# HKU-BAL/Clair3-RNA

Measured on AMD Instinct MI355X. Metric: candidate sites/sec (tensor build + inference), higher is better.
Workload: dtype f16 hi/lo split x3, f32 accumulate (fp32-equivalent); 1 GPU; synthetic ONT dRNA004 chr20 ~20x (BASELINE.json configs[1]); contig_len=64444167, chunks=13, channels=18, precision=f16x3, reads_per_rank=53937, exonic_bp_per_rank=1936903, parallelism=chunks sharded by contig, 1 rank(s), no collective, streams=2

## Files before the change

### clair3_rna_amd/csrc/net_kernels.hpp

```cpp
#pragma once
#include <hip/hip_runtime.h>
#include <mutex>
#include <chrono>
#include <type_traits>
#include <stdint.h>

#include <cmath>
#include <cstring>
#include <functional>
#include <string>
#include <vector>

#include "../../include/c3r.h"

namespace c3r {

typedef float floatx16 __attribute__((ext_vector_type(16)));
typedef float floatx4 __attribute__((ext_vector_type(4)));

constexpr int NET_H1 = 128;
constexpr int NET_H2 = 160;
constexpr int NET_T = C3R_WINDOW;
constexpr int NET_SITES = 32;
constexpr int LSTM_SB = 2;
constexpr int LSTM_SITES = NET_SITES * LSTM_SB;
#ifndef C3R_W8_PD
#define C3R_W8_PD 1
#endif
#ifndef C3R_W8_MAP
#define C3R_W8_MAP 0
#endif
#ifndef C3R_W8_PRIO
#define C3R_W8_PRIO 0
#endif
#ifndef C3R_DIR_ILV
#define C3R_DIR_ILV 1
#endif
constexpr int NET_FLAT = NET_T * 2 * NET_H2;
constexpr int NET_L4 = 128;

__device__ __forceinline__ float fast_sigmoid(float x) {
    return __builtin_amdgcn_rcpf(1.0f + __builtin_amdgcn_exp2f(-1.4426950408889634f * x));
}
__device__ __forceinline__ float fast_tanh(float x) {
    return fmaf(2.0f, __builtin_amdgcn_rcpf(1.0f + __builtin_amdgcn_exp2f(-2.8853900817779268f * x)), -1.0f);
}
__device__ __forceinline__ float gate_frac(float a, float b) {
    const float t = 1.0f + a;
    const float r = __builtin_amdgcn_rcpf(fmaf(t, b, t));
    return fmaf(-b, r, r);
}
__device__ __forceinline__ float selu(float x) {
    const float scale = 1.0507009873554805f, alpha = 1.6732632423543772f;
    return x > 0.f ? scale * x : scale * alpha * (__expf(x) - 1.0f);
}

template <int INP, int CIN, int H, bool INT_IN, int SB = 2, int ABL = 0>
__global__ __launch_bounds__(256, (SB == 1 ? 2 : 1)) void k_lstm(const void *__restrict__ xin, const float4 *__restrict__ Wp,
                                                                  const float *__restrict__ bp, float *__restrict__ y, int n,
                                                                  const int32_t *__restrict__ row_idx = nullptr ,
                                                                  int x16 = 0 ) {
    constexpr int NGX = INP / 8;
    constexpr int NGH = H / 8;
    constexpr int NG = NGX + NGH;
    constexpr int HP = H + 4;
    constexpr int NBLK = 4 * H / 32;
    constexpr int NT = NBLK / 4;
    constexpr int WG_SITES = 32 * SB;
    static_assert(INP % 16 == 0 && H % 32 == 0, "shape: even k-group counts for the ping-pong pipeline");
    __shared__ __attribute__((aligned(16))) float hbuf[2][WG_SITES][HP];

    const int tid = threadIdx.x, lane = tid & 63, wave = tid >> 6;
    const int j = lane & 31, hh = lane >> 5;
    const int dir = blockIdx.y;
    const int site0 = blockIdx.x * WG_SITES;

    const float4 *wl = Wp + ((size_t)(dir * 4 + wave) * NG) * NT * 64 + lane;
    float bias_a[NT];
#pragma unroll
    for (int tt = 0; tt < NT; ++tt) bias_a[tt] = hh == 0 ? bp[((size_t)dir * NBLK + wave * NT + tt) * 32 + j] : 0.f;

    float cst[NT][SB][4];
#pragma unroll
    for (int tt = 0; tt < NT; ++tt)
// ... 167 lines not shown
#define C3R_W8_ASYNC 1
#endif
__device__ __forceinline__ void lds_arrive(int *c) {
    __builtin_amdgcn_fence(__ATOMIC_RELEASE, "workgroup");
    if ((threadIdx.x & 63) == 0) atomicAdd(c, 1);
}
__device__ __forceinline__ void lds_wait(int *c, int target, int *tmo) {
    for (int it = 0; __atomic_load_n(c, __ATOMIC_RELAXED) < target; ++it) {
        if (it >= (1 << 24)) { if ((threadIdx.x & 63) == 0 && tmo) atomicOr(tmo, 1); break; }
        __builtin_amdgcn_s_sleep(1);
    }
    __builtin_amdgcn_fence(__ATOMIC_ACQUIRE, "workgroup");
}

#ifndef C3R_PROBE_Y1
#define C3R_PROBE_Y1 0
#endif
__host__ __device__ constexpr int w16_bias_row(int st, int q, int m) { return 8 * ((2 * q + st) & 3) + 4 * ((2 * q + st) >> 2) + m; }
template <int ABL = 0, bool RTS = false>
__global__ __launch_bounds__(512, 2) void k_lstm2_w16(const _Float16 *__restrict__ xin, const half8 *__restrict__ Wp,
                                                       const float *__restrict__ bp, int n, const half8 *__restrict__ W4p,
                                                       float *__restrict__ a4part, int nstride, float wsc_arg = WSCALE, float wun_arg = WUNSCALE, float wun4_arg = WUNSCALE,
                                                       int *tmo = nullptr ) {
    const float wsc = RTS ? wsc_arg : WSCALE, wun = RTS ? wun_arg : WUNSCALE, wun4 = RTS ? wun4_arg : WUNSCALE;
    constexpr int INP = 2 * NET_H1, H = NET_H2, NGX = INP / 32, NGH = H / 32, NG = NGX + NGH, NU = 2 * NG, HP = H + 8, NBLK = 4 * H / 32, NTQ = NBLK / 4;
    constexpr int SB = 4, WG_SITES = 16 * SB, KC = INP / 8, PD = C3R_W8_PD;
    static_assert(NTQ == 5 && NU == 26 && PD == 1, "3 + 2 tile split of a quarter, 26 (k-group, subtile) units, one unit of prefetch");
    __shared__ __attribute__((aligned(16))) _Float16 hb_hi[2][WG_SITES][HP];
    __shared__ __attribute__((aligned(16))) _Float16 hb_lo[2][WG_SITES][HP];
    __shared__ __attribute__((aligned(16))) _Float16 xs[2][KC][WG_SITES][8];
    __shared__ __attribute__((aligned(16))) float s_bias[NBLK][2][16];
    __shared__ int s_ctr[4];

    const int tid = threadIdx.x, lane = tid & 63, wave = tid >> 6;
    const int c16 = lane & 15, q4 = lane >> 4;
    const int sq = C3R_W8_MAP ? (wave >> 1) : (wave & 3);
    const bool heavy3 = C3R_W8_MAP ? !(wave & 1) : (wave < 4);
    const int dir = C3R_DIR_ILV ? blockIdx.x : blockIdx.y;
    const int site0 = (C3R_DIR_ILV ? blockIdx.y : blockIdx.x) * WG_SITES;
    const int ns = nstride ? nstride : n;
    const size_t plane_in = (size_t)ns * NET_T * INP;

    for (int i = tid; i < WG_SITES * HP; i += 512) { (&hb_hi[0][0][0])[i] = (_Float16)0.f; (&hb_lo[0][0][0])[i] = (_Float16)0.f; }
    for (int i = tid; i < NBLK * 32; i += 512) {
        const int T = i >> 5, st = (i >> 4) & 1, q = (i >> 2) & 3, m = i & 3;
        s_bias[T][st][4 * q + m] = wsc * bp[((size_t)dir * NBLK + T) * 32 + w16_bias_row(st, q, m)];
    }
    if (tid < 4) s_ctr[tid] = 0;

    int xsite = site0 + lane;
    if (xsite >= n) xsite = n - 1;
    auto dma_x = [&](int tt_) {
        typedef const _Float16 __attribute__((address_space(1))) *gp_t;
        typedef _Float16 __attribute__((address_space(3))) *lp_t;
#pragma unroll
        for (int r = 0; r < 2 * KC / 8; ++r) {
            const int row = wave * (2 * KC / 8) + r, pl = row / KC, kc = row % KC;
            const _Float16 *src = xin + (size_t)pl * plane_in + (((size_t)tt_ * KC + kc) * ns + xsite) * 8;
            __builtin_amdgcn_global_load_lds((gp_t)src, (lp_t)&xs[pl][kc][0][0], 16, 0, 0);
        }
    };
    auto dma_x16 = [&](int tt_) {
        typedef const _Float16 __attribute__((address_space(1))) *gp_t;
        typedef _Float16 __attribute__((address_space(3))) *lp_t;
#pragma unroll
        for (int r = 0; r < 2 * KC / 4; ++r) {
            const int row = (wave & 3) * (2 * KC / 4) + r, pl = row / KC, kc = row % KC;
            const _Float16 *src = xin + (size_t)pl * plane_in + (((size_t)tt_ * KC + kc) * ns + xsite) * 8;
            __builtin_amdgcn_global_load_lds((gp_t)src, (lp_t)&xs[pl][kc][0][0], 16, 0, 0);
        }
    };
    dma_x(dir ? NET_T - 1 : 0);
    asm volatile("s_waitcnt vmcnt(0)" ::: "memory");
    __syncthreads();

    auto body = [&](auto ntc, auto toffc, auto l4c) {
        constexpr int NT = decltype(ntc)::value, TOFF = decltype(toffc)::value;
        constexpr bool L4T = decltype(l4c)::value;
        constexpr int NTH = NT + (L4T ? 1 : 0);
        const half8 *wl = Wp + ((size_t)(dir * 4 + sq) * NU) * NTQ * 2 * 64 + (size_t)TOFF * 2 * 64 + lane;
        float cst[NT][2 * SB];
#pragma unroll
        for (int tt = 0; tt < NT; ++tt)
#pragma unroll
            for (int u = 0; u < 2 * SB; ++u) cst[tt][u] = 0.f;
        floatx4 facc[L4T ? 2 : 1][L4T ? SB : 1];
#pragma unroll
        for (int st = 0; st < (L4T ? 2 : 1); ++st)
#pragma unroll
            for (int sb = 0; sb < (L4T ? SB : 1); ++sb)
#pragma unroll
                for (int r = 0; r < 4; ++r) facc[st][sb][r] = 0.f;

        typedef const half8 __attribute__((address_space(1))) *gptr_t;
        for (int step = 0; step < NET_T; ++step) {
            const int t = dir ? NET_T - 1 - step : step;
            const int tprev = step ? (dir ? t + 1 : t - 1) : t;
            const int cur = step & 1, nxt = cur ^ 1;

            auto ldx = [&](int g, half8 (&bh)[SB], half8 (&bl)[SB]) {
#pragma unroll
                for (int sb = 0; sb < SB; ++sb) {
                    if ((ABL & 32) && g > 0) continue;
                    bh[sb] = *(const half8 *)&xs[0][4 * g + q4][16 * sb + c16][0];
                    bl[sb] = *(const half8 *)&xs[1][4 * g + q4][16 * sb + c16][0];
                }
            };
            auto ldh = [&](int g, half8 (&bh)[SB], half8 (&bl)[SB]) {
#pragma unroll
                for (int sb = 0; sb < SB; ++sb) {
                    if (ABL & 32) continue;
                    bh[sb] = *(const half8 *)&hb_hi[cur][16 * sb + c16][32 * g + 8 * q4];
                    bl[sb] = *(const half8 *)&hb_lo[cur][16 * sb + c16][32 * g + 8 * q4];
                }
            };
            auto ldw = [&](int u, half8 (&ah)[NTH], half8 (&al)[NTH]) {
                uintptr_t wbase = (uintptr_t)wl;
                asm volatile("" : "+v"(wbase));
                const gptr_t wg = (gptr_t)wbase + (size_t)((ABL & 1) ? 0 : u) * NTQ * 2 * 64;
#pragma unroll
                for (int tt = 0; tt < NT; ++tt) {
                    if ((ABL & 16) && u > 0) continue;
                    ah[tt] = wg[(tt * 2 + 0) * 64]; al[tt] = wg[(tt * 2 + 1) * 64];
                }
                if constexpr (L4T) {
                    if (u >= 2 * NGX && !((ABL & 16) && u > 2 * NGX)) {
                        uintptr_t w4base = (uintptr_t)(W4p + (((size_t)(dir * NET_T + tprev) * 4 + sq) * 2 * NGH) * 2 * 64 + lane);
                        asm volatile("" : "+v"(w4base));
                        const gptr_t w4 = (gptr_t)w4base + (size_t)(u - 2 * NGX) * 2 * 64;
                        ah[NT] = w4[0]; al[NT] = w4[64];
                    }
                }
            };

            if (C3R_W8_ASYNC && step > 0) lds_wait(&s_ctr[1], 4 * step, tmo);
            floatx4 acc[NT][2][SB];
#pragma unroll
            for (int tt = 0; tt < NT; ++tt)
#pragma unroll
                for (int st = 0; st < 2; ++st) {
                    const floatx4 b4 = *(const floatx4 *)&s_bias[sq * NTQ + TOFF + tt][st][4 * q4];
#pragma unroll
                    for (int sb = 0; sb < SB; ++sb) acc[tt][st][sb] = b4;
                }
            auto mma = [&](const half8 (&ah)[NTH], const half8 (&al)[NTH], const half8 (&bh)[SB], const half8 (&bl)[SB], auto stc, bool hpart) {
                constexpr int st = decltype(stc)::value;
#pragma unroll
                for (int tt = 0; tt < NT; ++tt)
#pragma unroll
                    for (int sb = 0; sb < SB; ++sb) acc[tt][st][sb] = __builtin_amdgcn_mfma_f32_16x16x32_f16(ah[tt], bh[sb], acc[tt][st][sb], 0, 0, 0);
                if (L4T && hpart) {
#pragma unroll
                    for (int sb = 0; sb < SB; ++sb) facc[L4T ? st : 0][L4T ? sb : 0] = __builtin_amdgcn_mfma_f32_16x16x32_f16(ah[L4T ? NT : 0], bh[sb], facc[L4T ? st : 0][L4T ? sb : 0], 0, 0, 0);
                }
#pragma unroll
                for (int tt = 0; tt < NT; ++tt)
#pragma unroll
                    for (int sb = 0; sb < SB; ++sb) acc[tt][st][sb] = __builtin_amdgcn_mfma_f32_16x16x32_f16(ah[tt], bl[sb], acc[tt][st][sb], 0, 0, 0);
                if (L4T && hpart) {
#pragma unroll
                    for (int sb = 0; sb < SB; ++sb) facc[L4T ? st : 0][L4T ? sb : 0] = __builtin_amdgcn_mfma_f32_16x16x32_f16(ah[L4T ? NT : 0], bl[sb], facc[L4T ? st : 0][L4T ? sb : 0], 0, 0, 0);
                }
#pragma unroll
// ... 26 lines not shown
            if constexpr (C3R_W8_ASYNC) lds_arrive(&s_ctr[0]); else __syncthreads();                              \
        }                                                                                                         \
    }
            C3R_LOAD(0);
            C3R_STEP(0) C3R_STEP(1) C3R_STEP(2) C3R_STEP(3) C3R_STEP(4) C3R_STEP(5) C3R_STEP(6) C3R_STEP(7) C3R_STEP(8) C3R_STEP(9)
            C3R_STEP(10) C3R_STEP(11) C3R_STEP(12) C3R_STEP(13) C3R_STEP(14) C3R_STEP(15) C3R_STEP(16) C3R_STEP(17) C3R_STEP(18)
            C3R_STEP(19) C3R_STEP(20) C3R_STEP(21) C3R_STEP(22) C3R_STEP(23) C3R_STEP(24) C3R_STEP(25)
            C3R_FENCE();
#undef C3R_STEP
#undef C3R_LOAD
#undef C3R_FENCE
            if constexpr (C3R_W8_ASYNC) {
                if (!L4T && step + 1 < NET_T) { lds_wait(&s_ctr[0], 8 * (step + 1), tmo); dma_x16(dir ? NET_T - 2 - step : step + 1); }
            } else if (step + 1 < NET_T && !(ABL & 64)) dma_x(dir ? NET_T - 2 - step : step + 1);
#pragma unroll
            for (int tt = 0; tt < NT; ++tt) {
                __builtin_amdgcn_sched_barrier(0);
                constexpr int NC = 2 * SB;
                const float K1 = -1.4426950408889634f * wun, K2 = -2.8853900817779268f * wun;
                float cq[NC], ei[NC], ef[NC], eg[NC], eo[NC], hval[NC];
#pragma unroll
                for (int u = 0; u < NC; ++u) cq[u] = cst[tt][u];
                if (ABL & 2) {
#pragma unroll
                    for (int u = 0; u < NC; ++u) hval[u] = acc[tt][u / SB][u % SB][0] + acc[tt][u / SB][u % SB][1] + acc[tt][u / SB][u % SB][2] + acc[tt][u / SB][u % SB][3];
                } else {
#pragma unroll
                    for (int u = 0; u < NC; ++u) ei[u] = fminf(__builtin_amdgcn_exp2f(K1 * acc[tt][u / SB][u % SB][0]), 1e18f);
#pragma unroll
                    for (int u = 0; u < NC; ++u) ef[u] = __builtin_amdgcn_exp2f(K1 * acc[tt][u / SB][u % SB][1]);
#pragma unroll
                    for (int u = 0; u < NC; ++u) eg[u] = fminf(__builtin_amdgcn_exp2f(K2 * acc[tt][u / SB][u % SB][2]), 1e18f);
#pragma unroll
                    for (int u = 0; u < NC; ++u) eo[u] = fminf(__builtin_amdgcn_exp2f(K1 * acc[tt][u / SB][u % SB][3]), 1e18f);
#pragma unroll
                    for (int u = 0; u < NC; ++u) ei[u] = gate_frac(ei[u], eg[u]);
#pragma unroll
                    for (int u = 0; u < NC; ++u) ef[u] = __builtin_amdgcn_rcpf(1.0f + ef[u]);
#pragma unroll
                    for (int u = 0; u < NC; ++u) cq[u] = fmaf(ef[u], cq[u], ei[u]);
#pragma unroll
                    for (int u = 0; u < NC; ++u) eg[u] = fminf(__builtin_amdgcn_exp2f(-2.8853900817779268f * cq[u]), 1e18f);
#pragma unroll
                    for (int u = 0; u < NC; ++u) hval[u] = gate_frac(eo[u], eg[u]);
                }
#pragma unroll
                for (int u = 0; u < NC; ++u) cst[tt][u] = cq[u];
#pragma unroll
                for (int sb = 0; sb < SB; ++sb) {
                    typedef _Float16 half2v __attribute__((ext_vector_type(2)));
                    half2v vh, vl;
#pragma unroll
                    for (int st = 0; st < 2; ++st) {
                        vh[st] = (_Float16)hval[SB * st + sb];
                        float d = hval[SB * st + sb] - (float)vh[st];
                        asm volatile("" : "+v"(d));
                        vl[st] = (_Float16)d;
                    }
                    *(half2v *)&hb_hi[nxt][16 * sb + c16][8 * (sq * NTQ + TOFF + tt) + 2 * q4] = vh;
                    *(half2v *)&hb_lo[nxt][16 * sb + c16][8 * (sq * NTQ + TOFF + tt) + 2 * q4] = vl;
                }
            }
            if constexpr (C3R_W8_ASYNC) {
                lds_arrive(&s_ctr[2]);
                if (!L4T && step + 1 < NET_T) { asm volatile("s_waitcnt vmcnt(0)" ::: "memory"); lds_arrive(&s_ctr[1]); }
            } else {
            asm volatile("s_waitcnt vmcnt(0)" ::: "memory");
            __syncthreads();
            }
        }
        if constexpr (L4T) {
            if constexpr (C3R_W8_ASYNC) lds_wait(&s_ctr[2], 8 * NET_T, tmo);
            const int tl = dir ? 0 : NET_T - 1, hbuf = NET_T & 1;
            const half8 *w4 = W4p + (((size_t)(dir * NET_T + tl) * 4 + sq) * 2 * NGH) * 2 * 64 + lane;
#pragma unroll 1
            for (int g = 0; g < NGH; ++g) {
                half8 b_h[SB], b_l[SB];
#pragma unroll
                for (int sb = 0; sb < SB; ++sb) {
                    b_h[sb] = *(const half8 *)&hb_hi[hbuf][16 * sb + c16][32 * g + 8 * q4];
                    b_l[sb] = *(const half8 *)&hb_lo[hbuf][16 * sb + c16][32 * g + 8 * q4];
                }
#pragma unroll
                for (int st = 0; st < 2; ++st) {
                    const half8 a_h = w4[(size_t)((2 * g + st) * 2 + 0) * 64], a_l = w4[(size_t)((2 * g + st) * 2 + 1) * 64];
#pragma unroll
                    for (int sb = 0; sb < SB; ++sb) facc[st][sb] = __builtin_amdgcn_mfma_f32_16x16x32_f16(a_h, b_h[sb], facc[st][sb], 0, 0, 0);
#pragma unroll
                    for (int sb = 0; sb < SB; ++sb) facc[st][sb] = __builtin_amdgcn_mfma_f32_16x16x32_f16(a_h, b_l[sb], facc[st][sb], 0, 0, 0);
#pragma unroll
                    for (int sb = 0; sb < SB; ++sb) facc[st][sb] = __builtin_amdgcn_mfma_f32_16x16x32_f16(a_l, b_h[sb], facc[st][sb], 0, 0, 0);
// ... 238 lines not shown
            constexpr int NTL = ((G) + PD >= NGX ? NTH : NT);                                                     \
            sched_interleave<NMM, NTL * ((((G) + PD) & 1) ? 3 : 1), SB * ((((G) + PD) & 1) ? 3 : 1)>();           \
        }                                                                                                         \
        if constexpr ((G) == NGX - 1) {                                                                           \
            C3R_FENCE();                                                                                          \
            if constexpr (C3R_W8_ASYNC) lds_arrive(&s_ctr[0]); else __syncthreads();             \
        }                                                                                                         \
    }
            if constexpr (PD > 0) { load(std::integral_constant<int, 0>{}, ah[0], bh[0]); }
            C3R_STEP(0) C3R_STEP(1) C3R_STEP(2) C3R_STEP(3) C3R_STEP(4) C3R_STEP(5) C3R_STEP(6) C3R_STEP(7) C3R_STEP(8) C3R_STEP(9)
            C3R_STEP(10) C3R_STEP(11) C3R_STEP(12) C3R_STEP(13) C3R_STEP(14) C3R_STEP(15) C3R_STEP(16) C3R_STEP(17) C3R_STEP(18)
            C3R_STEP(19) C3R_STEP(20) C3R_STEP(21) C3R_STEP(22) C3R_STEP(23) C3R_STEP(24) C3R_STEP(25)
            C3R_FENCE();
#undef C3R_STEP
#undef C3R_FENCE
            if constexpr (C3R_W8_ASYNC) {
                if (!L4T && step + 1 < NET_T) { lds_wait(&s_ctr[0], 8 * (step + 1), tmo); dma_x16(dir ? NET_T - 2 - step : step + 1); }
            } else if (step + 1 < NET_T) dma_x(dir ? NET_T - 2 - step : step + 1);
#pragma unroll
            for (int tt = 0; tt < NT; ++tt) {
                __builtin_amdgcn_sched_barrier(0);
                constexpr int NU = 4 * SB;
                constexpr float K1 = -1.4426950408889634f * WUNSCALE, K2 = -2.8853900817779268f * WUNSCALE;
                float cq[NU], ei[NU], ef[NU], eg[NU], eo[NU], hval[NU];
#pragma unroll
                for (int u = 0; u < NU; ++u) cq[u] = cst[tt][u >> 2][u & 3];
#pragma unroll
                for (int u = 0; u < NU; ++u) ei[u] = fminf(__builtin_amdgcn_exp2f(K1 * acc[tt][u >> 2][4 * (u & 3) + 0]), 1e18f);
#pragma unroll
                for (int u = 0; u < NU; ++u) ef[u] = __builtin_amdgcn_exp2f(K1 * acc[tt][u >> 2][4 * (u & 3) + 1]);
#pragma unroll
                for (int u = 0; u < NU; ++u) eg[u] = fminf(__builtin_amdgcn_exp2f(K2 * acc[tt][u >> 2][4 * (u & 3) + 2]), 1e18f);
#pragma unroll
                for (int u = 0; u < NU; ++u) eo[u] = fminf(__builtin_amdgcn_exp2f(K1 * acc[tt][u >> 2][4 * (u & 3) + 3]), 1e18f);
#pragma unroll
                for (int u = 0; u < NU; ++u) ei[u] = gate_frac(ei[u], eg[u]);
#pragma unroll
                for (int u = 0; u < NU; ++u) ef[u] = __builtin_amdgcn_rcpf(1.0f + ef[u]);
#pragma unroll
                for (int u = 0; u < NU; ++u) cq[u] = fmaf(ef[u], cq[u], ei[u]);
#pragma unroll
                for (int u = 0; u < NU; ++u) eg[u] = fminf(__builtin_amdgcn_exp2f(-2.8853900817779268f * cq[u]), 1e18f);
#pragma unroll
                for (int u = 0; u < NU; ++u) hval[u] = gate_frac(eo[u], eg[u]);
                const int T = sq * NTQ + TOFF + tt;
#pragma unroll
                for (int sb = 0; sb < SB; ++sb) {
#pragma unroll
                    for (int q = 0; q < 4; ++q) cst[tt][sb][q] = cq[4 * sb + q];
                    typedef _Float16 half4 __attribute__((ext_vector_type(4)));
                    half4 vh;
                    float lo[4];
#pragma unroll
                    for (int q = 0; q < 4; ++q) {
                        vh[q] = (_Float16)hval[4 * sb + q];
                        float d = hval[4 * sb + q] - (float)vh[q];
                        asm volatile("" : "+v"(d));
                        lo[q] = d * 262144.f;
                    }
                    *(half4 *)&hb_hi[nxt][32 * sb + j][8 * T + 4 * hh] = vh;
                    int w_lo = __builtin_amdgcn_cvt_pk_fp8_f32(lo[0], lo[1], 0, false);
                    w_lo = __builtin_amdgcn_cvt_pk_fp8_f32(lo[2], lo[3], w_lo, true);
                    int w_hi = __builtin_amdgcn_cvt_pk_fp8_f32(hval[4 * sb + 0] * 64.f, hval[4 * sb + 1] * 64.f, 0, false);
                    w_hi = __builtin_amdgcn_cvt_pk_fp8_f32(hval[4 * sb + 2] * 64.f, hval[4 * sb + 3] * 64.f, w_hi, true);
                    {
                    reinterpret_cast<int *>(&hq[nxt][T >> 2][0][(T & 3) >> 1][32 * sb + j])[2 * (T & 1) + hh] = w_lo;
                    reinterpret_cast<int *>(&hq[nxt][T >> 2][1][(T & 3) >> 1][32 * sb + j])[2 * (T & 1) + hh] = w_hi;
                    }
                }
            }
            if constexpr (C3R_W8_ASYNC) {
                lds_arrive(&s_ctr[2]);
                if (!L4T && step + 1 < NET_T) { asm volatile("s_waitcnt vmcnt(0)" ::: "memory"); lds_arrive(&s_ctr[1]); }
            } else {
            asm volatile("s_waitcnt vmcnt(0)" ::: "memory");
            __syncthreads();
            }
        }
        if constexpr (L4T) {
            if constexpr (C3R_W8_ASYNC) lds_wait(&s_ctr[2], 8 * NET_T, tmo);
            const int tl = dir ? 0 : NET_T - 1, hbuf = NET_T & 1;
            const half8 *w4 = W4p + (((size_t)(dir * NET_T + tl) * 4 + sq) * NGH) * 2 * 64 + lane;
            const intx8 *q4 = reinterpret_cast<const intx8 *>(W4q) + ((size_t)(dir * NET_T + tl) * 4 + sq) * NKBH * 64 + lane;
            const uint32_t *s4 = W4sc + ((size_t)(dir * NET_T + tl) * 4 + sq) * NK4L * 64 + lane;
            static_for<0, NKBH>([&](auto pc) {
                constexpr int P = decltype(pc)::value;
                const half8 a0 = w4[(size_t)((2 * P) * 2) * 64], a1 = w4[(size_t)((2 * P + 1) * 2) * 64];
                const intx8 aq = ld_q((g8_t)(q4 + (size_t)P * 64));
                const int scl = (int)s4[(size_t)(P / 4) * 64];
#pragma unroll
                for (int sb = 0; sb < SB; ++sb) {
                    const half8 b0 = *(const half8 *)&hb_hi[hbuf][32 * sb + j][16 * (2 * P) + 8 * hh];
// ... 3 lines not shown
                    facc[sb] = __builtin_amdgcn_mfma_f32_32x32x16_f16(a0, b0, facc[sb], 0, 0, 0);
                    facc[sb] = __builtin_amdgcn_mfma_f32_32x32x16_f16(a1, b1, facc[sb], 0, 0, 0);
                    facc[sb] = __builtin_amdgcn_mfma_scale_f32_32x32x64_f8f6f4(aq, bq, facc[sb], 0, 0, P % 4, scl, 0, sbc);
                }
            });
#pragma unroll
            for (int sb = 0; sb < SB; ++sb) {
                const int sidx = site0 + 32 * sb + j;
                if (sidx < n) {
#pragma unroll
                    for (int q = 0; q < 4; ++q) {
                        float4 v = make_float4(facc[sb][4 * q] * WUNSCALE, facc[sb][4 * q + 1] * WUNSCALE, facc[sb][4 * q + 2] * WUNSCALE,
                                               facc[sb][4 * q + 3] * WUNSCALE);
                        *(float4 *)(a4part + ((size_t)sidx * 2 + dir) * NET_L4 + 32 * sq + 8 * q + 4 * hh) = v;
                    }
                }
            }
        }
    };
#ifndef C3R_MX_PRIO
#define C3R_MX_PRIO 0
#endif
    if (C3R_MX_PRIO == 1 && heavy3) __builtin_amdgcn_s_setprio(1);
    if (C3R_MX_PRIO == 2 && !heavy3) __builtin_amdgcn_s_setprio(1);
    if (heavy3) body(std::integral_constant<int, 3>{}, std::integral_constant<int, 0>{}, std::false_type{});
    else body(std::integral_constant<int, 2>{}, std::integral_constant<int, 3>{}, std::true_type{});
}

template <int CIN, bool YQ = false, bool RTS = false>
__global__ __launch_bounds__(1024) void k_lstm1_rs(const void *__restrict__ xin_v, const half8 *__restrict__ Wp, _Float16 *__restrict__ y, int n, int nstride,
                                                   const int32_t *__restrict__ row_idx ,
                                                   float wun_arg = WUNSCALE ,
                                                   int x16 = 0 ) {
    const int32_t *__restrict__ xin = (const int32_t *)xin_v;
    const int16_t *__restrict__ xin16 = (const int16_t *)xin_v;
    const float wun = RTS ? wun_arg : WUNSCALE;
    constexpr int H = NET_H1, NGX = 2, NGH = H / 16, NG = NGX + NGH, HP = H + 8, NTQ = 4, WG_SITES = 64, HV = H / 8, XP = 40;
    constexpr int NPC = (CIN + 1) / 2;
    static_assert(CIN % 2 == 0 && CIN < 32 && WG_SITES * NPC <= 1024, "even channel count, one free slot for the bias, one x piece per thread");
    typedef _Float16 half4 __attribute__((ext_vector_type(4)));
    __shared__ __attribute__((aligned(16))) _Float16 hb_hi[2][WG_SITES][HP];
    __shared__ __attribute__((aligned(16))) _Float16 hb_lo[2][WG_SITES][HP];
    __shared__ __attribute__((aligned(16))) _Float16 xs[4][2][WG_SITES][XP];
    __shared__ int s_xlvl[NET_T];
    __shared__ __attribute__((aligned(16))) float4 s_c[16][2][64];
    const int tid = threadIdx.x, lane = tid & 63, blk = tid >> 6;
    const int j = lane & 31, hh = lane >> 5;
    const int dir = C3R_DIR_ILV ? blockIdx.x : blockIdx.y;
    const int site0 = (C3R_DIR_ILV ? blockIdx.y : blockIdx.x) * WG_SITES;
    const size_t plane_out = (size_t)nstride * NET_T * 2 * H;

    for (int i = tid; i < WG_SITES * HP; i += 1024) { (&hb_hi[0][0][0])[i] = (_Float16)0.f; (&hb_lo[0][0][0])[i] = (_Float16)0.f; }
    for (int i = tid; i < 2 * WG_SITES * XP; i += 1024) {
        (&xs[0][0][0][0])[i] = ((i % XP) == CIN) ? (_Float16)1.f : (_Float16)0.f;
        (&xs[1][0][0][0])[i] = (_Float16)0.f; (&xs[2][0][0][0])[i] = (_Float16)0.f; (&xs[3][0][0][0])[i] = (_Float16)0.f;
    }
    if (tid < NET_T) s_xlvl[tid] = 0;

    half8 wh[NG], wl[NG];
    {
        const half8 *wb = Wp + (((size_t)(dir * 4 + (blk >> 2)) * NG) * NTQ + (blk & 3)) * 2 * 64 + lane;
#pragma unroll
        for (int g = 0; g < NG; ++g) { wh[g] = wb[((size_t)g * NTQ * 2 + 0) * 64]; wl[g] = wb[((size_t)g * NTQ * 2 + 1) * 64]; }
    }
    s_c[blk][0][lane] = make_float4(0.f, 0.f, 0.f, 0.f);
    s_c[blk][1][lane] = make_float4(0.f, 0.f, 0.f, 0.f);

    typedef int int2v __attribute__((ext_vector_type(2)));
    int2v xr = {0, 0};
    const bool xmine = tid < WG_SITES * NPC;
    uint32_t xrow = 0;
    if (xmine) {
        int sj = site0 + tid / NPC;
        if (sj >= n) sj = n - 1;
        if (row_idx) sj = row_idx[sj];
        xrow = (uint32_t)sj * (uint32_t)(NET_T * CIN) + 2u * (uint32_t)(tid % NPC);
    }
    auto x_fetch = [&](int tt_) {
        if (xmine) {
            if (x16) { const int pr = *(const int *)(xin16 + (size_t)(xrow + (uint32_t)(tt_ * CIN))); xr[0] = (int)(int16_t)(pr & 0xffff); xr[1] = pr >> 16; }
            else xr = *(const int2v *)(xin + (size_t)(xrow + (uint32_t)(tt_ * CIN)));
        }
    };
    auto x_store = [&](int buf, int step_) {
        if (xmine) {
            typedef _Float16 half2v __attribute__((ext_vector_type(2)));
            half2v vrh, vrl;
            int r[2] = {xr[0], xr[1]}, any_t = 0;
            const int site = tid / NPC, slot = 2 * (tid % NPC);
            if (!x16) {
                half2v vth, vtl;
#pragma unroll
                for (int e = 0; e < 2; ++e) {
                    const int T = (r[e] >> 16) + ((r[e] >> 15) & 1);
                    r[e] = (int)((uint32_t)r[e] - ((uint32_t)T << 16));
                    vth[e] = (_Float16)(float)T;
                    vtl[e] = (_Float16)(float)(T - (int)(float)vth[e]);
                    any_t |= T;
                }
                *(half2v *)&xs[2][buf][site][slot] = vth; *(half2v *)&xs[3][buf][site][slot] = vtl;
            }
            vrh[0] = (_Float16)(float)r[0]; vrh[1] = (_Float16)(float)r[1];
            const int rl0 = r[0] - (int)(float)vrh[0], rl1 = r[1] - (int)(float)vrh[1];
            vrl[0] = (_Float16)(float)rl0; vrl[1] = (_Float16)(float)rl1;
            const int any_rl = rl0 | rl1;
            *(half2v *)&xs[0][buf][site][slot] = vrh;
            *(half2v *)&xs[1][buf][site][slot] = vrl;
            if (any_rl | any_t) atomicMax(&s_xlvl[step_], any_t ? 2 : 1);
        }
    };
    __syncthreads();
    x_fetch(dir ? NET_T - 1 : 0);
    x_store(0, 0);
    __syncthreads();
#ifndef C3R_L1_K8
#define C3R_L1_K8 1
#endif
#ifndef C3R_L1_RS_PRIO
#define C3R_L1_RS_PRIO 0
#endif
    if (C3R_L1_RS_PRIO > 0 && blk >= C3R_L1_RS_PRIO) __builtin_amdgcn_s_setprio(1);

    auto one_step = [&](const int step, auto deep_c) {
        constexpr bool DEEP = decltype(deep_c)::value;
        const int t = dir ? NET_T - 1 - step : step;
        const int cur = step & 1, nxt = cur ^ 1;
#pragma unroll
        for (int sb = 0; sb < 2; ++sb) {
            const _Float16 *xb = &xs[0][cur][32 * sb + j][8 * hh];
            constexpr int XPART = 2 * WG_SITES * XP;
            if (sb == 1 && step + 1 < NET_T) x_fetch(dir ? NET_T - 2 - step : step + 1);
            floatx16 acc;
#pragma unroll
            for (int r = 0; r < 16; ++r) acc[r] = 0.f;
            if constexpr (DEEP) {
                if (__builtin_amdgcn_readfirstlane(s_xlvl[step]) == 2) {
#pragma unroll
                    for (int g = 0; g < NGX; ++g) {
                        const half8 th = *(const half8 *)(xb + 2 * XPART + 16 * g), tl = *(const half8 *)(xb + 3 * XPART + 16 * g);
                        acc = __builtin_amdgcn_mfma_f32_32x32x16_f16(wh[g], th, acc, 0, 0, 0);
                        acc = __builtin_amdgcn_mfma_f32_32x32x16_f16(wl[g], th, acc, 0, 0, 0);
                        acc = __builtin_amdgcn_mfma_f32_32x32x16_f16(wh[g], tl, acc, 0, 0, 0);
                        acc = __builtin_amdgcn_mfma_f32_32x32x16_f16(wl[g], tl, acc, 0, 0, 0);
                    }
#pragma unroll
                    for (int r = 0; r < 16; ++r) acc[r] *= 65536.f;
                }
#pragma unroll
                for (int g = 0; g < NGX; ++g) {
                    const half8 rl = *(const half8 *)(xb + XPART + 16 * g);
                    acc = __builtin_amdgcn_mfma_f32_32x32x16_f16(wh[g], rl, acc, 0, 0, 0);
                    acc = __builtin_amdgcn_mfma_f32_32x32x16_f16(wl[g], rl, acc, 0, 0, 0);
                }
            }
            half8 bh[2], bl[2];
            auto ldb = [&](auto gc, half8 &h, half8 &l) {
                constexpr int G = decltype(gc)::value;
                if constexpr (G < NGX) h = *(const half8 *)(xb + 16 * G);
                else { h = *(const half8 *)&hb_hi[cur][32 * sb + j][16 * (G - NGX) + 8 * hh]; l = *(const half8 *)&hb_lo[cur][32 * sb + j][16 * (G - NGX) + 8 * hh]; }
            };
            if constexpr (!DEEP) ldb(std::integral_constant<int, 0>{}, bh[0], bl[0]);
            static_for<0, NG>([&](auto gc) {
                constexpr int G = decltype(gc)::value;
                if constexpr (DEEP) ldb(std::integral_constant<int, G>{}, bh[G & 1], bl[G & 1]);
                else if constexpr (G + 1 < NG) ldb(std::integral_constant<int, G + 1>{}, bh[(G + 1) & 1], bl[(G + 1) & 1]);
                if constexpr (C3R_L1_K8 && G == NGX - 1 && CIN + 1 <= 16 + 4) {
                    const half4 a_h = __builtin_shufflevector(wh[G], wh[G], 0, 1, 2, 3), a_l = __builtin_shufflevector(wl[G], wl[G], 0, 1, 2, 3);
                    const half4 b_h = __builtin_shufflevector(bh[G & 1], bh[G & 1], 0, 1, 2, 3);
                    acc = __builtin_amdgcn_mfma_f32_32x32x8f16(a_h, b_h, acc, 0, 0, 0);
                    acc = __builtin_amdgcn_mfma_f32_32x32x8f16(a_l, b_h, acc, 0, 0, 0);
                } else {
                acc = __builtin_amdgcn_mfma_f32_32x32x16_f16(wh[G], bh[G & 1], acc, 0, 0, 0);
                acc = __builtin_amdgcn_mfma_f32_32x32x16_f16(wl[G], bh[G & 1], acc, 0, 0, 0);
                if constexpr (G >= NGX) acc = __builtin_amdgcn_mfma_f32_32x32x16_f16(wh[G], bl[G & 1], acc, 0, 0, 0);
                }
            });
            const float K1 = -1.4426950408889634f * wun, K2 = -2.8853900817779268f * wun;
            float ei[4], ef[4], eg[4], eo[4], cq[4], hval[4];
            {
                const float4 c4 = s_c[blk][sb][lane];
                cq[0] = c4.x; cq[1] = c4.y; cq[2] = c4.z; cq[3] = c4.w;
            }
#pragma unroll
            for (int u = 0; u < 4; ++u) ei[u] = fminf(__builtin_amdgcn_exp2f(K1 * acc[4 * u + 0]), 1e18f);
#pragma unroll
            for (int u = 0; u < 4; ++u) ef[u] = __builtin_amdgcn_exp2f(K1 * acc[4 * u + 1]);
#pragma unroll
            for (int u = 0; u < 4; ++u) eg[u] = fminf(__builtin_amdgcn_exp2f(K2 * acc[4 * u + 2]), 1e18f);
#pragma unroll
            for (int u = 0; u < 4; ++u) eo[u] = fminf(__builtin_amdgcn_exp2f(K1 * acc[4 * u + 3]), 1e18f);
#pragma unroll
            for (int u = 0; u < 4; ++u) ei[u] = gate_frac(ei[u], eg[u]);
#pragma unroll
            for (int u = 0; u < 4; ++u) ef[u] = __builtin_amdgcn_rcpf(1.0f + ef[u]);
#pragma unroll
            for (int u = 0; u < 4; ++u) cq[u] = fmaf(ef[u], cq[u], ei[u]);
#pragma unroll
            for (int u = 0; u < 4; ++u) eg[u] = fminf(__builtin_amdgcn_exp2f(-2.8853900817779268f * cq[u]), 1e18f);
#pragma unroll
            for (int u = 0; u < 4; ++u) hval[u] = gate_frac(eo[u], eg[u]);
            s_c[blk][sb][lane] = make_float4(cq[0], cq[1], cq[2], cq[3]);
            half4 vh, vl;
            float lo[4];
#pragma unroll
            for (int q = 0; q < 4; ++q) {
                vh[q] = (_Float16)hval[q];
                float d = hval[q] - (float)vh[q];
                asm volatile("" : "+v"(d));
                vl[q] = (_Float16)d;
                lo[q] = d * 262144.f;
            }
            *(half4 *)&hb_hi[nxt][32 * sb + j][8 * blk + 4 * hh] = vh;
            *(half4 *)&hb_lo[nxt][32 * sb + j][8 * blk + 4 * hh] = vl;
            _Float16 *yp = y + ((size_t)t * (2 * HV) + dir * HV + blk) * nstride * 8 + (uint32_t)(site0 + 32 * sb + j) * 8 + 4 * hh;
            *(half4 *)yp = vh;
            if constexpr (!YQ) {
                if (!(C3R_PROBE_Y1 && (blk & 1))) *(half4 *)(yp + plane_out) = vl;
            } else {
                int w_lo = __builtin_amdgcn_cvt_pk_fp8_f32(lo[0], lo[1], 0, false);
                w_lo = __builtin_amdgcn_cvt_pk_fp8_f32(lo[2], lo[3], w_lo, true);
                int w_hi = __builtin_amdgcn_cvt_pk_fp8_f32(hval[0] * 64.f, hval[1] * 64.f, 0, false);
                w_hi = __builtin_amdgcn_cvt_pk_fp8_f32(hval[2] * 64.f, hval[3] * 64.f, w_hi, true);
                const int row0 = (dir * 4 + (blk >> 2)) * 4 + ((blk & 3) >> 1);
                _Float16 *qp = y + plane_out + ((size_t)t * (2 * HV) + row0) * nstride * 8 + (uint32_t)(site0 + 32 * sb + j) * 8 + 4 * (blk & 1) + 2 * hh;
                *(int *)qp = w_lo;
                *(int *)(qp + (size_t)2 * nstride * 8) = w_hi;
            }
        }
        if (step + 1 < NET_T) x_store(nxt, step + 1);
        __syncthreads();
    };
    int step = 0;
    for (; step < NET_T; ++step) {
        if (__builtin_amdgcn_readfirstlane(s_xlvl[step])) break;
        one_step(step, std::false_type{});
    }
    for (; step < NET_T; ++step) one_step(step, std::true_type{});
}

__global__ __launch_bounds__(256) void k_fc4(const float *__restrict__ y2, const float4 *__restrict__ Wp,
                                             const float *__restrict__ bias, float *__restrict__ a4, int n) {
    constexpr int NG = NET_FLAT / 8;
    const int tid = threadIdx.x, lane = tid & 63, wave = tid >> 6;
    const int j = lane & 31, hh = lane >> 5;
    const int site0 = blockIdx.x * NET_SITES;
    int s = site0 + j; if (s >= n) s = n - 1;
    const float *xrow = y2 + (size_t)s * NET_FLAT + 4 * hh;
    const float4 *wl = Wp + (size_t)wave * NG * 64 + lane;
    floatx16 acc0, acc1;
#pragma unroll
    for (int r = 0; r < 16; ++r) { acc0[r] = 0.f; acc1[r] = 0.f; }
#pragma unroll 4
    for (int g = 0; g < NG; g += 2) {
        const float4 b0 = *(const float4 *)(xrow + 8 * g);
        const float4 b1 = *(const float4 *)(xrow + 8 * g + 8);
        const float4 a0 = wl[(size_t)g * 64];
        const float4 a1 = wl[(size_t)(g + 1) * 64];
        acc0 = __builtin_amdgcn_mfma_f32_32x32x2f32(a0.x, b0.x, acc0, 0, 0, 0);
        acc1 = __builtin_amdgcn_mfma_f32_32x32x2f32(a1.x, b1.x, acc1, 0, 0, 0);
        acc0 = __builtin_amdgcn_mfma_f32_32x32x2f32(a0.y, b0.y, acc0, 0, 0, 0);
        acc1 = __builtin_amdgcn_mfma_f32_32x32x2f32(a1.y, b1.y, acc1, 0, 0, 0);
        acc0 = __builtin_amdgcn_mfma_f32_32x32x2f32(a0.z, b0.z, acc0, 0, 0, 0);
// ... 650 lines not shown
```

Baseline: 8.461 million sites/s.

## Scalarize LSTM address math, pack hi/lo split, and fence cell ops

Weight, output and x-load base pointers in the LSTM kernels are moved into scalar registers, and only a per-lane offset is added, which is meant to cut VGPR pressure and per-lane 64-bit address arithmetic. LDS read and write pointers are kept as running pointers that toggle between ping-pong buffers each step instead of being recomputed. The hi/lo fp16 split now uses packed conversion and v_fma_mix to compute the residual, and a redundant fminf clamp on the output gate is removed. Compiler fences around cell-state ops and sched_barriers around operand prefetch are added to steer instruction scheduling, at some risk of constraining the scheduler.

```diff
diff --git a/clair3_rna_amd/csrc/net_kernels.hpp b/clair3_rna_amd/csrc/net_kernels.hpp
--- a/clair3_rna_amd/csrc/net_kernels.hpp
+++ b/clair3_rna_amd/csrc/net_kernels.hpp
@@ -50,6 +50,22 @@
     const float r = __builtin_amdgcn_rcpf(fmaf(t, b, t));
     return fmaf(-b, r, r);
 }
+__device__ __forceinline__ float cell_fence(float x) {
+    asm("" : "+v"(x));
+    return x;
+}
+typedef _Float16 half2v __attribute__((ext_vector_type(2)));
+typedef float float2v __attribute__((ext_vector_type(2)));
+__device__ __forceinline__ void split_h2(float h0, float h1, half2v &hi, half2v &lo, float &d0, float &d1) {
+    asm("" : "+v"(h0));
+    asm("" : "+v"(h1));
+    const float2v h = {h0, h1};
+    hi = __builtin_convertvector(h, half2v);
+    asm("v_fma_mix_f32 %0, -%1, 1.0, %2 op_sel_hi:[1,1,0]" : "=v"(d0) : "v"(hi), "v"(h0));
+    asm("v_fma_mix_f32 %0, -%1, 1.0, %2 op_sel:[1,0,0] op_sel_hi:[1,1,0]" : "=v"(d1) : "v"(hi), "v"(h1));
+    const float2v d = {d0, d1};
+    lo = __builtin_convertvector(d, half2v);
+}
 __device__ __forceinline__ float selu(float x) {
     const float scale = 1.0507009873554805f, alpha = 1.6732632423543772f;
     return x > 0.f ? scale * x : scale * alpha * (__expf(x) - 1.0f);
@@ -283,7 +299,8 @@
     __shared__ __attribute__((aligned(16))) float s_bias[NBLK][2][16];
     __shared__ int s_ctr[4];
 
-    const int tid = threadIdx.x, lane = tid & 63, wave = tid >> 6;
+    const int tid = threadIdx.x, lane = tid & 63;
+    const int wave = __builtin_amdgcn_readfirstlane(tid >> 6);
     const int c16 = lane & 15, q4 = lane >> 4;
     const int sq = C3R_W8_MAP ? (wave >> 1) : (wave & 3);
     const bool heavy3 = C3R_W8_MAP ? !(wave & 1) : (wave < 4);
@@ -329,7 +346,7 @@
         constexpr int NT = decltype(ntc)::value, TOFF = decltype(toffc)::value;
         constexpr bool L4T = decltype(l4c)::value;
         constexpr int NTH = NT + (L4T ? 1 : 0);
-        const half8 *wl = Wp + ((size_t)(dir * 4 + sq) * NU) * NTQ * 2 * 64 + (size_t)TOFF * 2 * 64 + lane;
+        const half8 *wl = Wp + ((size_t)(dir * 4 + sq) * NU) * NTQ * 2 * 64 + (size_t)TOFF * 2 * 64;
         float cst[NT][2 * SB];
 #pragma unroll
         for (int tt = 0; tt < NT; ++tt)
@@ -344,6 +361,7 @@
                 for (int r = 0; r < 4; ++r) facc[st][sb][r] = 0.f;
 
         typedef const half8 __attribute__((address_space(1))) *gptr_t;
+        const uint32_t wlane = (uint32_t)lane;
         for (int step = 0; step < NET_T; ++step) {
             const int t = dir ? NET_T - 1 - step : step;
             const int tprev = step ? (dir ? t + 1 : t - 1) : t;
@@ -366,20 +384,18 @@
                 }
             };
             auto ldw = [&](int u, half8 (&ah)[NTH], half8 (&al)[NTH]) {
-                uintptr_t wbase = (uintptr_t)wl;
-                asm volatile("" : "+v"(wbase));
-                const gptr_t wg = (gptr_t)wbase + (size_t)((ABL & 1) ? 0 : u) * NTQ * 2 * 64;
+                gptr_t wg = (gptr_t)wl + (size_t)((ABL & 1) ? 0 : u) * NTQ * 2 * 64;
+                asm volatile("" : "+s"(wg));
 #pragma unroll
                 for (int tt = 0; tt < NT; ++tt) {
                     if ((ABL & 16) && u > 0) continue;
-                    ah[tt] = wg[(tt * 2 + 0) * 64]; al[tt] = wg[(tt * 2 + 1) * 64];
+                    ah[tt] = wg[(tt * 2 + 0) * 64 + wlane]; al[tt] = wg[(tt * 2 + 1) * 64 + wlane];
                 }
                 if constexpr (L4T) {
                     if (u >= 2 * NGX && !((ABL & 16) && u > 2 * NGX)) {
-                        uintptr_t w4base = (uintptr_t)(W4p + (((size_t)(dir * NET_T + tprev) * 4 + sq) * 2 * NGH) * 2 * 64 + lane);
-                        asm volatile("" : "+v"(w4base));
-                        const gptr_t w4 = (gptr_t)w4base + (size_t)(u - 2 * NGX) * 2 * 64;
-                        ah[NT] = w4[0]; al[NT] = w4[64];
+                        gptr_t w4 = (gptr_t)(W4p + (((size_t)(dir * NET_T + tprev) * 4 + sq) * 2 * NGH) * 2 * 64) + (size_t)(u - 2 * NGX) * 2 * 64;
+                        asm volatile("" : "+s"(w4));
+                        ah[NT] = w4[wlane]; al[NT] = w4[64 + wlane];
                     }
                 }
             };
@@ -472,13 +488,13 @@
 #pragma unroll
                     for (int u = 0; u < NC; ++u) eg[u] = fminf(__builtin_amdgcn_exp2f(K2 * acc[tt][u / SB][u % SB][2]), 1e18f);
 #pragma unroll
-                    for (int u = 0; u < NC; ++u) eo[u] = fminf(__builtin_amdgcn_exp2f(K1 * acc[tt][u / SB][u % SB][3]), 1e18f);
-#pragma unroll
-                    for (int u = 0; u < NC; ++u) ei[u] = gate_frac(ei[u], eg[u]);
+                    for (int u = 0; u < NC; ++u) eo[u] = __builtin_amdgcn_exp2f(K1 * acc[tt][u / SB][u % SB][3]);
+#pragma unroll
+                    for (int u = 0; u < NC; ++u) ei[u] = cell_fence(gate_frac(ei[u], eg[u]));
 #pragma unroll
                     for (int u = 0; u < NC; ++u) ef[u] = __builtin_amdgcn_rcpf(1.0f + ef[u]);
 #pragma unroll
-                    for (int u = 0; u < NC; ++u) cq[u] = fmaf(ef[u], cq[u], ei[u]);
+                    for (int u = 0; u < NC; ++u) cq[u] = cell_fence(fmaf(ef[u], cq[u], ei[u]));
 #pragma unroll
                     for (int u = 0; u < NC; ++u) eg[u] = fminf(__builtin_amdgcn_exp2f(-2.8853900817779268f * cq[u]), 1e18f);
 #pragma unroll
@@ -488,15 +504,9 @@
                 for (int u = 0; u < NC; ++u) cst[tt][u] = cq[u];
 #pragma unroll
                 for (int sb = 0; sb < SB; ++sb) {
-                    typedef _Float16 half2v __attribute__((ext_vector_type(2)));
                     half2v vh, vl;
-#pragma unroll
-                    for (int st = 0; st < 2; ++st) {
-                        vh[st] = (_Float16)hval[SB * st + sb];
-                        float d = hval[SB * st + sb] - (float)vh[st];
-                        asm volatile("" : "+v"(d));
-                        vl[st] = (_Float16)d;
-                    }
+                    float d0, d1;
+                    split_h2(hval[sb], hval[SB + sb], vh, vl, d0, d1);
                     *(half2v *)&hb_hi[nxt][16 * sb + c16][8 * (sq * NTQ + TOFF + tt) + 2 * q4] = vh;
                     *(half2v *)&hb_lo[nxt][16 * sb + c16][8 * (sq * NTQ + TOFF + tt) + 2 * q4] = vl;
                 }
@@ -801,13 +811,13 @@
 #pragma unroll
                 for (int u = 0; u < NU; ++u) eg[u] = fminf(__builtin_amdgcn_exp2f(K2 * acc[tt][u >> 2][4 * (u & 3) + 2]), 1e18f);
 #pragma unroll
-                for (int u = 0; u < NU; ++u) eo[u] = fminf(__builtin_amdgcn_exp2f(K1 * acc[tt][u >> 2][4 * (u & 3) + 3]), 1e18f);
-#pragma unroll
-                for (int u = 0; u < NU; ++u) ei[u] = gate_frac(ei[u], eg[u]);
+                for (int u = 0; u < NU; ++u) eo[u] = __builtin_amdgcn_exp2f(K1 * acc[tt][u >> 2][4 * (u & 3) + 3]);
+#pragma unroll
+                for (int u = 0; u < NU; ++u) ei[u] = cell_fence(gate_frac(ei[u], eg[u]));
 #pragma unroll
                 for (int u = 0; u < NU; ++u) ef[u] = __builtin_amdgcn_rcpf(1.0f + ef[u]);
 #pragma unroll
-                for (int u = 0; u < NU; ++u) cq[u] = fmaf(ef[u], cq[u], ei[u]);
+                for (int u = 0; u < NU; ++u) cq[u] = cell_fence(fmaf(ef[u], cq[u], ei[u]));
 #pragma unroll
                 for (int u = 0; u < NU; ++u) eg[u] = fminf(__builtin_amdgcn_exp2f(-2.8853900817779268f * cq[u]), 1e18f);
 #pragma unroll
@@ -818,15 +828,13 @@
 #pragma unroll
                     for (int q = 0; q < 4; ++q) cst[tt][sb][q] = cq[4 * sb + q];
                     typedef _Float16 half4 __attribute__((ext_vector_type(4)));
-                    half4 vh;
+                    half2v vh01, vh23, vl01, vl23;
                     float lo[4];
-#pragma unroll
-                    for (int q = 0; q < 4; ++q) {
-                        vh[q] = (_Float16)hval[4 * sb + q];
-                        float d = hval[4 * sb + q] - (float)vh[q];
-                        asm volatile("" : "+v"(d));
-                        lo[q] = d * 262144.f;
-                    }
+                    split_h2(hval[4 * sb + 0], hval[4 * sb + 1], vh01, vl01, lo[0], lo[1]);
+                    split_h2(hval[4 * sb + 2], hval[4 * sb + 3], vh23, vl23, lo[2], lo[3]);
+                    const half4 vh = __builtin_shufflevector(vh01, vh23, 0, 1, 2, 3);
+#pragma unroll
+                    for (int q = 0; q < 4; ++q) lo[q] *= 262144.f;
                     *(half4 *)&hb_hi[nxt][32 * sb + j][8 * T + 4 * hh] = vh;
                     int w_lo = __builtin_amdgcn_cvt_pk_fp8_f32(lo[0], lo[1], 0, false);
                     w_lo = __builtin_amdgcn_cvt_pk_fp8_f32(lo[2], lo[3], w_lo, true);
@@ -896,25 +904,23 @@
                                                    const int32_t *__restrict__ row_idx ,
                                                    float wun_arg = WUNSCALE ,
                                                    int x16 = 0 ) {
-    const int32_t *__restrict__ xin = (const int32_t *)xin_v;
-    const int16_t *__restrict__ xin16 = (const int16_t *)xin_v;
     const float wun = RTS ? wun_arg : WUNSCALE;
     constexpr int H = NET_H1, NGX = 2, NGH = H / 16, NG = NGX + NGH, HP = H + 8, NTQ = 4, WG_SITES = 64, HV = H / 8, XP = 40;
     constexpr int NPC = (CIN + 1) / 2;
     static_assert(CIN % 2 == 0 && CIN < 32 && WG_SITES * NPC <= 1024, "even channel count, one free slot for the bias, one x piece per thread");
     typedef _Float16 half4 __attribute__((ext_vector_type(4)));
-    __shared__ __attribute__((aligned(16))) _Float16 hb_hi[2][WG_SITES][HP];
-    __shared__ __attribute__((aligned(16))) _Float16 hb_lo[2][WG_SITES][HP];
+    __shared__ __attribute__((aligned(16))) _Float16 hb[2][2][WG_SITES][HP];
     __shared__ __attribute__((aligned(16))) _Float16 xs[4][2][WG_SITES][XP];
     __shared__ int s_xlvl[NET_T];
     __shared__ __attribute__((aligned(16))) float4 s_c[16][2][64];
-    const int tid = threadIdx.x, lane = tid & 63, blk = tid >> 6;
+    const int tid = threadIdx.x, lane = tid & 63;
+    const int blk = __builtin_amdgcn_readfirstlane(tid >> 6);
     const int j = lane & 31, hh = lane >> 5;
     const int dir = C3R_DIR_ILV ? blockIdx.x : blockIdx.y;
     const int site0 = (C3R_DIR_ILV ? blockIdx.y : blockIdx.x) * WG_SITES;
     const size_t plane_out = (size_t)nstride * NET_T * 2 * H;
 
-    for (int i = tid; i < WG_SITES * HP; i += 1024) { (&hb_hi[0][0][0])[i] = (_Float16)0.f; (&hb_lo[0][0][0])[i] = (_Float16)0.f; }
+    for (int i = tid; i < 2 * WG_SITES * HP; i += 1024) (&hb[0][0][0][0])[i] = (_Float16)0.f;
     for (int i = tid; i < 2 * WG_SITES * XP; i += 1024) {
         (&xs[0][0][0][0])[i] = ((i % XP) == CIN) ? (_Float16)1.f : (_Float16)0.f;
         (&xs[1][0][0][0])[i] = (_Float16)0.f; (&xs[2][0][0][0])[i] = (_Float16)0.f; (&xs[3][0][0][0])[i] = (_Float16)0.f;
@@ -940,10 +946,13 @@
         if (row_idx) sj = row_idx[sj];
         xrow = (uint32_t)sj * (uint32_t)(NET_T * CIN) + 2u * (uint32_t)(tid % NPC);
     }
+    uint32_t xesz = x16 ? 2u : 4u;
+    asm volatile("" : "+s"(xesz));
     auto x_fetch = [&](int tt_) {
         if (xmine) {
-            if (x16) { const int pr = *(const int *)(xin16 + (size_t)(xrow + (uint32_t)(tt_ * CIN))); xr[0] = (int)(int16_t)(pr & 0xffff); xr[1] = pr >> 16; }
-            else xr = *(const int2v *)(xin + (size_t)(xrow + (uint32_t)(tt_ * CIN)));
+            const char *xa = (const char *)xin_v + (uint64_t)(xrow + (uint32_t)(tt_ * CIN)) * xesz;
+            if (x16) { const int pr = *(const int *)xa; xr[0] = (int)(int16_t)(pr & 0xffff); xr[1] = pr >> 16; }
+            else xr = *(const int2v *)xa;
         }
     };
     auto x_store = [&](int buf, int step_) {
@@ -984,15 +993,29 @@
 #define C3R_L1_RS_PRIO 0
 #endif
     if (C3R_L1_RS_PRIO > 0 && blk >= C3R_L1_RS_PRIO) __builtin_amdgcn_s_setprio(1);
+    typedef const char __attribute__((address_space(3))) *lds_t;
+    typedef char __attribute__((address_space(3))) *ldsw_t;
+    typedef const half8 __attribute__((address_space(3))) *lds_h8;
+    constexpr int XBUF = WG_SITES * XP * 2, HBUF = 2 * WG_SITES * HP * 2, HLO = WG_SITES * HP * 2, XPARTB = 2 * XBUF;
+    lds_t xrd = (lds_t)&xs[0][0][j][8 * hh];
+    lds_t hrd = (lds_t)&hb[0][0][j][8 * hh];
+    ldsw_t hwr = (ldsw_t)&hb[1][0][j][8 * blk + 4 * hh];
+    const ldsw_t scp = (ldsw_t)&s_c[blk][0][lane];
+    asm volatile("" : "+v"(xrd), "+v"(hrd), "+v"(hwr));
 
     auto one_step = [&](const int step, auto deep_c) {
         constexpr bool DEEP = decltype(deep_c)::value;
         const int t = dir ? NET_T - 1 - step : step;
         const int cur = step & 1, nxt = cur ^ 1;
+        typedef _Float16 __attribute__((address_space(1))) *gh_t;
+        typedef half4 __attribute__((address_space(1))) *gh4_t;
+        gh_t yrow = (gh_t)(y + ((size_t)t * (2 * HV) + dir * HV + blk) * nstride * 8 + (size_t)site0 * 8);
+        asm volatile("" : "+s"(yrow));
+        const uint32_t ylane = (uint32_t)(j * 8 + 4 * hh);
 #pragma unroll
         for (int sb = 0; sb < 2; ++sb) {
-            const _Float16 *xb = &xs[0][cur][32 * sb + j][8 * hh];
-            constexpr int XPART = 2 * WG_SITES * XP;
+            const lds_t xb = xrd + 32 * sb * XP * 2;
+            const lds_t hb_r = hrd + 32 * sb * HP * 2;
             if (sb == 1 && step + 1 < NET_T) x_fetch(dir ? NET_T - 2 - step : step + 1);
             floatx16 acc;
 #pragma unroll
@@ -1001,7 +1024,7 @@
                 if (__builtin_amdgcn_readfirstlane(s_xlvl[step]) == 2) {
 #pragma unroll
                     for (int g = 0; g < NGX; ++g) {
-                        const half8 th = *(const half8 *)(xb + 2 * XPART + 16 * g), tl = *(const half8 *)(xb + 3 * XPART + 16 * g);
+                        const half8 th = *(lds_h8)(xb + 2 * XPARTB + 32 * g), tl = *(lds_h8)(xb + 3 * XPARTB + 32 * g);
                         acc = __builtin_amdgcn_mfma_f32_32x32x16_f16(wh[g], th, acc, 0, 0, 0);
                         acc = __builtin_amdgcn_mfma_f32_32x32x16_f16(wl[g], th, acc, 0, 0, 0);
                         acc = __builtin_amdgcn_mfma_f32_32x32x16_f16(wh[g], tl, acc, 0, 0, 0);
@@ -1012,7 +1035,7 @@
                 }
 #pragma unroll
                 for (int g = 0; g < NGX; ++g) {
-                    const half8 rl = *(const half8 *)(xb + XPART + 16 * g);
+                    const half8 rl = *(lds_h8)(xb + XPARTB + 32 * g);
                     acc = __builtin_amdgcn_mfma_f32_32x32x16_f16(wh[g], rl, acc, 0, 0, 0);
                     acc = __builtin_amdgcn_mfma_f32_32x32x16_f16(wl[g], rl, acc, 0, 0, 0);
                 }
@@ -1020,14 +1043,18 @@
             half8 bh[2], bl[2];
             auto ldb = [&](auto gc, half8 &h, half8 &l) {
                 constexpr int G = decltype(gc)::value;
-                if constexpr (G < NGX) h = *(const half8 *)(xb + 16 * G);
-                else { h = *(const half8 *)&hb_hi[cur][32 * sb + j][16 * (G - NGX) + 8 * hh]; l = *(const half8 *)&hb_lo[cur][32 * sb + j][16 * (G - NGX) + 8 * hh]; }
+                if constexpr (G < NGX) h = *(lds_h8)(xb + 32 * G);
+                else { h = *(lds_h8)(hb_r + 32 * (G - NGX)); l = *(lds_h8)(hb_r + HLO + 32 * (G - NGX)); }
             };
             if constexpr (!DEEP) ldb(std::integral_constant<int, 0>{}, bh[0], bl[0]);
             static_for<0, NG>([&](auto gc) {
                 constexpr int G = decltype(gc)::value;
                 if constexpr (DEEP) ldb(std::integral_constant<int, G>{}, bh[G & 1], bl[G & 1]);
-                else if constexpr (G + 1 < NG) ldb(std::integral_constant<int, G + 1>{}, bh[(G + 1) & 1], bl[(G + 1) & 1]);
+                else {
+                    __builtin_amdgcn_sched_barrier(0);
+                    if constexpr (G + 1 < NG) ldb(std::integral_constant<int, G + 1>{}, bh[(G + 1) & 1], bl[(G + 1) & 1]);
+                    __builtin_amdgcn_sched_barrier(0);
+                }
                 if constexpr (C3R_L1_K8 && G == NGX - 1 && CIN + 1 <= 16 + 4) {
                     const half4 a_h = __builtin_shufflevector(wh[G], wh[G], 0, 1, 2, 3), a_l = __builtin_shufflevector(wl[G], wl[G], 0, 1, 2, 3);
                     const half4 b_h = __builtin_shufflevector(bh[G & 1], bh[G & 1], 0, 1, 2, 3);
@@ -1042,8 +1069,8 @@
             const float K1 = -1.4426950408889634f * wun, K2 = -2.8853900817779268f * wun;
             float ei[4], ef[4], eg[4], eo[4], cq[4], hval[4];
             {
-                const float4 c4 = s_c[blk][sb][lane];
-                cq[0] = c4.x; cq[1] = c4.y; cq[2] = c4.z; cq[3] = c4.w;
+                const floatx4 c4 = *(floatx4 __attribute__((address_space(3))) *)(scp + sb * 64 * 16);
+                cq[0] = c4[0]; cq[1] = c4[1]; cq[2] = c4[2]; cq[3] = c4[3];
             }
 #pragma unroll
             for (int u = 0; u < 4; ++u) ei[u] = fminf(__builtin_amdgcn_exp2f(K1 * acc[4 * u + 0]), 1e18f);
@@ -1052,46 +1079,51 @@
 #pragma unroll
             for (int u = 0; u < 4; ++u) eg[u] = fminf(__builtin_amdgcn_exp2f(K2 * acc[4 * u + 2]), 1e18f);
 #pragma unroll
-            for (int u = 0; u < 4; ++u) eo[u] = fminf(__builtin_amdgcn_exp2f(K1 * acc[4 * u + 3]), 1e18f);
-#pragma unroll
-            for (int u = 0; u < 4; ++u) ei[u] = gate_frac(ei[u], eg[u]);
+            for (int u = 0; u < 4; ++u) eo[u] = __builtin_amdgcn_exp2f(K1 * acc[4 * u + 3]);
+#pragma unroll
+            for (int u = 0; u < 4; ++u) ei[u] = cell_fence(gate_frac(ei[u], eg[u]));
 #pragma unroll
             for (int u = 0; u < 4; ++u) ef[u] = __builtin_amdgcn_rcpf(1.0f + ef[u]);
 #pragma unroll
-            for (int u = 0; u < 4; ++u) cq[u] = fmaf(ef[u], cq[u], ei[u]);
+            for (int u = 0; u < 4; ++u) cq[u] = cell_fence(fmaf(ef[u], cq[u], ei[u]));
 #pragma unroll
             for (int u = 0; u < 4; ++u) eg[u] = fminf(__builtin_amdgcn_exp2f(-2.8853900817779268f * cq[u]), 1e18f);
 #pragma unroll
             for (int u = 0; u < 4; ++u) hval[u] = gate_frac(eo[u], eg[u]);
-            s_c[blk][sb][lane] = make_float4(cq[0], cq[1], cq[2], cq[3]);
-            half4 vh, vl;
+            *(floatx4 __attribute__((address_space(3))) *)(scp + sb * 64 * 16) = floatx4{cq[0], cq[1], cq[2], cq[3]};
+            half2v vh01, vh23, vl01, vl23;
             float lo[4];
-#pragma unroll
-            for (int q = 0; q < 4; ++q) {
-                vh[q] = (_Float16)hval[q];
-                float d = hval[q] - (float)vh[q];
-                asm volatile("" : "+v"(d));
-                vl[q] = (_Float16)d;
-                lo[q] = d * 262144.f;
-            }
-            *(half4 *)&hb_hi[nxt][32 * sb + j][8 * blk + 4 * hh] = vh;
-            *(half4 *)&hb_lo[nxt][32 * sb + j][8 * blk + 4 * hh] = vl;
-            _Float16 *yp = y + ((size_t)t * (2 * HV) + dir * HV + blk) * nstride * 8 + (uint32_t)(site0 + 32 * sb + j) * 8 + 4 * hh;
-            *(half4 *)yp = vh;
+            split_h2(hval[0], hval[1], vh01, vl01, lo[0], lo[1]);
+            split_h2(hval[2], hval[3], vh23, vl23, lo[2], lo[3]);
+            const half4 vh = __builtin_shufflevector(vh01, vh23, 0, 1, 2, 3), vl = __builtin_shufflevector(vl01, vl23, 0, 1, 2, 3);
+#pragma unroll
+            for (int q = 0; q < 4; ++q) lo[q] *= 262144.f;
+            *(half4 __attribute__((address_space(3))) *)(hwr + 32 * sb * HP * 2) = vh;
+            *(half4 __attribute__((address_space(3))) *)(hwr + 32 * sb * HP * 2 + HLO) = vl;
+            const gh_t yp = yrow + (size_t)(ylane + 32 * sb * 8);
+            *(gh4_t)yp = vh;
             if constexpr (!YQ) {
-                if (!(C3R_PROBE_Y1 && (blk & 1))) *(half4 *)(yp + plane_out) = vl;
+                if (!(C3R_PROBE_Y1 && (blk & 1))) *(gh4_t)(yrow + plane_out + (size_t)(ylane + 32 * sb * 8)) = vl;
             } else {
                 int w_lo = __builtin_amdgcn_cvt_pk_fp8_f32(lo[0], lo[1], 0, false);
                 w_lo = __builtin_amdgcn_cvt_pk_fp8_f32(lo[2], lo[3], w_lo, true);
                 int w_hi = __builtin_amdgcn_cvt_pk_fp8_f32(hval[0] * 64.f, hval[1] * 64.f, 0, false);
                 w_hi = __builtin_amdgcn_cvt_pk_fp8_f32(hval[2] * 64.f, hval[3] * 64.f, w_hi, true);
                 const int row0 = (dir * 4 + (blk >> 2)) * 4 + ((blk & 3) >> 1);
-                _Float16 *qp = y + plane_out + ((size_t)t * (2 * HV) + row0) * nstride * 8 + (uint32_t)(site0 + 32 * sb + j) * 8 + 4 * (blk & 1) + 2 * hh;
-                *(int *)qp = w_lo;
-                *(int *)(qp + (size_t)2 * nstride * 8) = w_hi;
+                gh_t qrow = (gh_t)(y + plane_out + ((size_t)t * (2 * HV) + row0) * nstride * 8 + (size_t)site0 * 8 + 4 * (blk & 1));
+                asm volatile("" : "+s"(qrow));
+                typedef int __attribute__((address_space(1))) *gi_t;
+                const uint32_t qlane = (uint32_t)(j * 8 + 2 * hh + 32 * sb * 8);
+                *(gi_t)(qrow + (size_t)qlane) = w_lo;
+                *(gi_t)(qrow + (size_t)2 * nstride * 8 + (size_t)qlane) = w_hi;
             }
         }
         if (step + 1 < NET_T) x_store(nxt, step + 1);
+        {
+            const int sg = cur ? -1 : 1;
+            xrd += sg * XBUF; hrd += sg * HBUF; hwr -= sg * HBUF;
+            asm volatile("" : "+v"(xrd), "+v"(hrd), "+v"(hwr));
+        }
         __syncthreads();
     };
     int step = 0;
```

New measurement: 8.923 million sites/s (median of 6 runs). +5.5%, better.
